# rccohn/AMPIS

Hardware: AMD Instinct MI355X
Metric: images/sec Mask R-CNN R50-FPN @1024x1024 inference (higher is better)
Workload: dtype f32 (convs: f16x3 split-operand MFMA -- 22-bit operands, exact products, fp32 accumulate); 1 GPU; BASELINE configs[1]: R50-FPN inference, batch=8 synthetic 1024x1024 micrographs per GPU, K=2, 1000 proposals/img, TEST.DETECTIONS_PER_IMAGE=200, seeded random-init weights, outputs on the host: boxes, scores, classes and every mask as its COCO compressed-RLE counts string (encoded on the device); batch_per_gpu=8, global_batch=8, parallelism=image-parallel replicas x1, no data-path collective

## Files before the change

ampis_amd/_lib.py:

```python
import ctypes as C
import os

_HERE = os.path.dirname(os.path.abspath(__file__))
LIB_PATH = os.path.join(_HERE, "lib", "libampis_hip.so")


class AmpError(RuntimeError):
    pass


class ConvDesc(C.Structure):
    _fields_ = [(n, C.c_int) for n in
                ("B", "H", "W", "Cin", "Cout", "KH", "KW", "stride", "pad", "relu", "res_mode", "out_mode")]


class RpnLevels(C.Structure):
    _fields_ = [("nlevels", C.c_int), ("A", C.c_int), ("ld", C.c_int), ("pred", C.c_void_p * 5),
                ("h", C.c_int * 5), ("w", C.c_int * 5), ("stride", C.c_int * 5), ("anchor_size", C.c_int * 5)]


class FpnFeats(C.Structure):
    _fields_ = [("feat", C.c_void_p * 4), ("h", C.c_int * 4), ("w", C.c_int * 4), ("stride", C.c_int * 4),
                ("C", C.c_int)]

# ... 66 lines not shown
        "amp_prof_launches": ([vp, C.POINTER(ProfLaunch), i, C.POINTER(i)], i),
        "amp_timer_stop": ([vp, C.POINTER(f)], i),
        "amp_destroy": ([vp], None),
        "amp_sync": ([vp], i),
        "amp_malloc": ([vp, C.c_size_t, C.POINTER(vp)], i),
        "amp_free": ([vp, vp], i),
        "amp_memcpy_h2d": ([vp, vp, vp, C.c_size_t], i),
        "amp_memcpy_d2h": ([vp, vp, vp, C.c_size_t], i),
        "amp_memset": ([vp, vp, i, C.c_size_t], i),
        "amp_conv2d_nhwc": ([vp, C.POINTER(ConvDesc), vp, vp, vp, vp, vp, vp], i),
        "amp_conv2d_nhwc_ex": ([vp, C.POINTER(ConvDesc), vp, vp, vp, vp, vp, vp, vp], i),
        "amp_conv2d_nhwc_fmt": ([vp, C.POINTER(ConvDesc), vp, vp, vp, vp, vp, vp, i], i),
        "amp_unsplit_rows": ([vp, vp, C.c_longlong, i, vp], i),
        "amp_group_expand_weights": ([vp, vp, i, i, i, i, vp], i),
        "amp_resize_scratch_bytes": ([i, i, i, i], C.c_size_t),
        "amp_resize_bilinear_u8": ([vp, vp, i, i, vp, i, i, vp], i),
        "amp_resize_flip_u8": ([vp, vp, i, i, vp, i, i, i, i, vp], i),
        "amp_compact_dets": ([vp, i, i, vp, vp, vp, vp, vp, vp, vp, vp], i),
        "amp_set_conv_mode": ([vp, i], i),
        "amp_get_conv_mode": ([vp], i),
        "amp_conv_range_flag": ([vp, i, C.POINTER(C.c_int)], i),
        "amp_split_weights": ([vp, vp, C.c_longlong, i, vp], i),
        "amp_bottleneck64_tail": ([vp, i, i, i, vp, vp, vp, vp, vp, vp, vp, i, vp, vp], i),
        "amp_conv2d_grouped_nhwc": ([vp, C.POINTER(ConvDesc), i, vp, vp, vp, vp, vp, vp], i),
        "amp_conv2d_grouped_nhwc_fmt": ([vp, C.POINTER(ConvDesc), i, vp, vp, vp, vp, vp, vp, i], i),
        "amp_conv_wgrad_scratch_floats": ([C.POINTER(ConvDesc)], C.c_size_t),
        "amp_conv2d_wgrad": ([vp, C.POINTER(ConvDesc), vp, vp, vp, vp, vp, i], i),
        "amp_conv2d_wgrad_scaled": ([vp, C.POINTER(ConvDesc), vp, vp, vp, vp, vp, i, i, i], i),
        "amp_colsum": ([vp, vp, i, i, vp, vp, i], i),
        "amp_dgrad_weights": ([vp, vp, vp, i, i, i, i, vp], i),
        "amp_dgrad_weights_split": ([vp, vp, vp, i, i, i, i, vp], i),
        "amp_preprocess": ([vp, vp, i, i, i, i, i, C.POINTER(f), C.POINTER(f), vp, vp], i),
        "amp_model_set_image_sizes": ([vp, vp, i], i),
        "amp_maxpool3x3s2": ([vp, vp, i, i, i, i, vp], i),
        "amp_subsample2": ([vp, vp, i, i, i, i, vp], i),
        "amp_rpn_topk": ([vp, C.POINTER(RpnLevels), i, i, vp, i, vp, vp, vp], i),
        "amp_rpn_decode": ([vp, C.POINTER(RpnLevels), i, i, vp, vp, vp, i, i, i, vp, vp, vp], i),
        "amp_rpn_decode_sized": ([vp, C.POINTER(RpnLevels), i, i, vp, vp, vp, i, i, vp, i, vp, vp, vp], i),
        "amp_sort_gather": ([vp, i, i, i, vp, vp, vp, vp, vp, vp, vp, vp, vp], i),
        "amp_sort_gather_n": ([vp, i, i, i, vp, vp, vp, vp, vp, vp, vp, vp, vp, vp], i),
        "amp_nms": ([vp, i, i, vp, vp, vp, f, i, vp, vp, vp], i),
        "amp_rpn_nms_scratch_words": ([i, i, i], C.c_size_t),
        "amp_rpn_nms_levels": ([vp, i, i, i, i, vp, vp, vp, f, i, vp, vp, vp, vp, vp, vp, vp], i),
        "amp_roi_align": ([vp, C.POINTER(FpnFeats), vp, vp, vp, i, i, vp, vp], i),
        "amp_roi_align_fmt": ([vp, C.POINTER(FpnFeats), vp, vp, vp, i, i, vp, vp, i], i),
        "amp_box_candidates": ([vp, vp, i, vp, vp, i, i, i, C.POINTER(f), f, i, i, vp, vp, i, vp, vp], i),
# ... 239 lines not shown
```

ampis_amd/csrc/common.h:

```cpp
#pragma once
#include <hip/hip_runtime.h>
#ifdef __HIPCC__
#include <hip/hip_ext.h>
#endif
#include <stdint.h>
#include <stdio.h>
#include <algorithm>
#include <string>

#include "../../include/ampis_hip.h"

namespace amp {

void set_error(const char* fmt, ...);

#define AMP_HIP_CHECK(expr)                                                         \
    do {                                                                            \
        hipError_t _e = (expr);                                                     \
        if (_e != hipSuccess) {                                                     \
            amp::set_error("%s:%d: %s -> %s", __FILE__, __LINE__, #expr,            \
                           hipGetErrorString(_e));                                  \
            return AMP_ERR_HIP;                                                     \
        }                                                                           \
    } while (0)
// ... 152 lines not shown
                       float* dense_boxes, unsigned long long* keys, int ccap, int* cand_count, int* overflow);
struct WeightJob {
    const float* w;
    const float* scale;
    unsigned int* out;
    int N, KH, KW, C;
    int transpose;
};
int weight_jobs_run(amp_ctx* ctx, const WeightJob* jobs_dev, const void* chunks_dev, int nchunks);
int sgd_chunks_run(amp_ctx* ctx, const unsigned long long* chunks_dev, int nchunks, float* p, const float* g, float* v, float lr,
                   float momentum, float weight_decay, float grad_scale);
int wgrad_async_begin(amp_ctx* ctx, float* scratch1);
int wgrad_async_join(amp_ctx* ctx);
int wgrad_async_end(amp_ctx* ctx);
int roi_align_bwd_run(amp_ctx* ctx, float* const dfeat[4], const int fh[4], const int fw[4], const int stride[4], int C, const float* rois,
                      const int* batch_idx, int R, int P, const float* dout, int B, int init);
int upsample2_bwd_run(amp_ctx* ctx, const float* dfine, float* dcoarse, int B, int Hc, int Wc, int C, int init);
int maxpool_run(amp_ctx* ctx, const float* x, int B, int H, int W, int C, float* y, int y_split);
int compact_dets_run(amp_ctx* ctx, int B, int D, const int* det_count, const float* det_boxes, const float* det_scores, const int* det_classes,
                     float* boxes, float* scores, int* classes, int* batch, int* n_total );
int stem_pool_run(amp_ctx* ctx, int B, int H, int W, const float* x, int x_split, const float* w_split, const float* scale, const float* shift,
                  float* pool, int pool_split);
int conv_c64_fused3_run(amp_ctx* ctx, int B, int H, int W, const float* x_split, const float* w2_split, const float* scale2, const float* shift2,
                        const float* w3_split, const float* scale3, const float* shift3, int C3, const float* res_split, float* y_split);
bool stem_pool_applies(amp_ctx* ctx, const float* w_split);
bool stem_u8_applies(amp_ctx* ctx, const float* w_split);
int stem_pool_u8_run(amp_ctx* ctx, const uint8_t* img, int B, int H, int W, int Hp, int Wp, const float mean[3], const float std_[3],
                     const int* img_hw, const float* w_split, const float* scale, const float* shift, float* pool, int pool_split);
int preprocess_run(amp_ctx* ctx, const uint8_t* img_bgr, int B, int H, int W, int Hp, int Wp, const float mean[3], const float std[3],
                   const int* img_hw, float* out, int out_split);
}
```

ampis_amd/csrc/conv.hip:

```cpp
#include "common.h"
#include <type_traits>

namespace {

typedef float f32x4 __attribute__((ext_vector_type(4)));
typedef float f32x16 __attribute__((ext_vector_type(16)));
typedef _Float16 f16x8 __attribute__((ext_vector_type(8)));
typedef _Float16 f16x2 __attribute__((ext_vector_type(2)));
typedef _Float16 f16x4 __attribute__((ext_vector_type(4)));
typedef unsigned int u32x4 __attribute__((ext_vector_type(4)));
constexpr float LO_SCALE = 2048.0f;

constexpr int BK = 32;
constexpr int LDS_LD = 36;

struct ConvArgs {
    const float* x;
    const float* w;
    const float* scale;
    const float* shift;
    const float* res;
    const float* mask;
    float* y;
    int B, H, W, Cin;
// ... 345 lines not shown
                }
                if (a.relu) o = fmaxf(o, 0.f);
                const _Float16 hh = (_Float16)o;
                hi[q] = hh;
                lo[q] = (_Float16)((o - (float)hh) * LO_SCALE);
            }
            if (mv[t]) {
                char* base = reinterpret_cast<char*>(a.y + yrow[t]) + col_b;
                *reinterpret_cast<f16x8*>(base) = hi;
                *reinterpret_cast<f16x8*>(base + 64) = lo;
            }
        }
        if (CHECK && bad) atomicOr(a.range_flag, 1);
    }
}

__device__ __forceinline__ int swap_channel(int w) {
    const int j = w >> 4, q = (w >> 2) & 3, e = w & 3;
    return 32 * (j >> 1) + 8 * q + 4 * (j & 1) + e;
}

typedef float f32x2 __attribute__((ext_vector_type(2)));

template <bool SPATIAL, bool CHECK, int MBR, bool AFFINE_LDS = false, bool PLAIN = false>
__device__ __forceinline__ void conv_epilogue_direct_rows(const ConvArgs& a, f32x4 (&acc)[MBR][4], int lane, const int (&mrow_in)[MBR], int nw0,
                                                          const float* lsc = nullptr, const float* lsh = nullptr, int nrel0 = 0) {
    const int lq = lane >> 4;
    const bool has_res = !PLAIN && a.res_mode != 0, has_mask = !PLAIN && a.mask != nullptr;
    const bool deconv = SPATIAL && a.out_mode == 1;
    const int C2 = a.Cout >> 2;
    const int tap = deconv ? nw0 / C2 : 0, ncol0 = deconv ? nw0 - tap * C2 : nw0;
    const int yld = deconv ? C2 : a.Cout;
    f32x2 sc[2][4], sh[2][4];
    size_t colb[2];
#pragma unroll
    for (int g = 0; g < 2; ++g) {
        const int n = nw0 + 32 * g + 8 * lq;
        const int nc = ncol0 + 32 * g + 8 * lq;
        colb[g] = (size_t)(nc >> 5) * 128 + (size_t)(nc & 31) * 2;
#pragma unroll
        for (int p = 0; p < 4; ++p) {
            if constexpr (AFFINE_LDS) {
                const int nr = nrel0 + 32 * g + 8 * lq + 2 * p;
                sc[g][p] = f32x2{lsc[nr], lsc[nr + 1]};
                sh[g][p] = f32x2{lsh[nr], lsh[nr + 1]};
            } else {
                sc[g][p] = a.scale ? f32x2{a.scale[n + 2 * p], a.scale[n + 2 * p + 1]} : f32x2{1.f, 1.f};
                sh[g][p] = a.shift ? f32x2{a.shift[n + 2 * p], a.shift[n + 2 * p + 1]} : f32x2{0.f, 0.f};
            }
// ... 78 lines not shown
                f32x2 o = v * sc[g][p] + sh[g][p];
                if (has_res) {
                    const f32x2 r1 = {(float)rh[g][2 * p], (float)rh[g][2 * p + 1]};
                    const f32x2 r2 = {(float)rl[g][2 * p], (float)rl[g][2 * p + 1]};
                    o = o + (r1 + r2 * (1.0f / LO_SCALE));
                }
                if (a.relu) { o[0] = fmaxf(o[0], 0.f); o[1] = fmaxf(o[1], 0.f); }
                if (has_mask) {
                    const f32x2 mk = f32x2{(float)mh[g][2 * p], (float)mh[g][2 * p + 1]} + f32x2{(float)ml[g][2 * p], (float)ml[g][2 * p + 1]} * (1.0f / LO_SCALE);
                    o[0] = mk[0] > 0.f ? o[0] : 0.f;
                    o[1] = mk[1] > 0.f ? o[1] : 0.f;
                }
                const f16x2 h = __builtin_convertvector(o, f16x2);
                const f32x2 hf = {(float)h[0], (float)h[1]};
                const f32x2 l = __builtin_elementwise_fma(hf, f32x2{-LO_SCALE, -LO_SCALE}, o * LO_SCALE);
                const f16x2 lh = __builtin_convertvector(l, f16x2);
                hi[2 * p] = h[0]; hi[2 * p + 1] = h[1];
                lo[2 * p] = lh[0]; lo[2 * p + 1] = lh[1];
            }
            if (mv) {
                char* base = reinterpret_cast<char*>(a.y + yrow) + colb[g];
                *reinterpret_cast<f16x8*>(base) = hi;
                *reinterpret_cast<f16x8*>(base + 64) = lo;
            }
        }
    }
    if (CHECK && (!(chk[0] == 0.f) || !(chk[1] == 0.f))) atomicOr(a.range_flag, 1);
}

template <bool SPATIAL, bool CHECK>
__device__ __forceinline__ void conv_epilogue_direct(const ConvArgs& a, f32x4 (&acc)[4][4], int lane, int mw0, int nw0) {
    const int l15 = lane & 15;
    const int mrows[4] = {mw0 + l15, mw0 + 16 + l15, mw0 + 32 + l15, mw0 + 48 + l15};
    conv_epilogue_direct_rows<SPATIAL, CHECK, 4>(a, acc, lane, mrows, nw0);
}

template <int WTM, int WTN, bool SPATIAL, bool CHECK>
__device__ __forceinline__ void conv_epilogue_swapped(const ConvArgs& a, f32x4 (&acc)[4][4], float* lds, int wave, int lane, int mw0, int nw0) {
    const int l15 = lane & 15, lq = lane >> 4;
    constexpr int SLD = WTN + 4;
    float* stage = lds + wave * (WTM * SLD);
#pragma unroll
    for (int i = 0; i < 4; ++i)
#pragma unroll
        for (int j = 0; j < 4; ++j)
            *reinterpret_cast<f32x4*>(stage + (i * 16 + l15) * SLD + 32 * (j >> 1) + 8 * lq + 4 * (j & 1)) = acc[i][j];
// ... 1395 lines not shown
            int mrows[2];
#pragma unroll
            for (int i = 0; i < 2; ++i) {
                const int oy = oyw + 2 * h + i, ox = ox0 + l15;
                mrows[i] = (oy < a.Ho && ox < a.Wo) ? (b * a.Ho + oy) * a.Wo + ox : a.M;
            }
            conv_epilogue_direct_rows<false, true, 2>(a, reinterpret_cast<f32x4 (&)[2][4]>(acc[2 * h]), lane, mrows, n0 + wn * 64);
        }
    }
#ifdef AMP_STAMP
    if (lane == 0)
        for (int q = 0; q < 8; ++q) atomicAdd(&g_stamp[wave * 8 + q], (unsigned long long)st_acc[q]);
#endif
}

struct Fuse3Args {
    const float* w3;
    const float* scale3;
    const float* shift3;
    const float* res;
    float* y;
    int C3;
    unsigned int w3_bytes;
};
template <bool DIAG, bool FUSE3 = false>
__global__ __launch_bounds__(256, 2) void conv3x3_c64_kernel(const ConvArgs a, const unsigned int x_bytes, const unsigned int w_bytes, const int tiles_x, const int tiles_y, const Fuse3Args f3) {
    constexpr int TH = 8, TW = 16, PH = TH + 2, PW = TW + 2, NPIX = PH * PW;
    constexpr int ROWF = 64;
    constexpr int NINST = NPIX / 4;
    static_assert(NPIX % 4 == 0, "patch pixels per DMA instruction");
    __shared__ __attribute__((aligned(16))) float lds[NPIX * ROWF + 2 * 64 * ROWF];
    float* patch = lds;
    float* wbuf = lds + NPIX * ROWF;
    const int tid = threadIdx.x, lane = tid & 63;
    const int wave = __builtin_amdgcn_readfirstlane(tid >> 6);
    const int l15 = lane & 15, lq = lane >> 4;
    int t = amp::xcd_remap(blockIdx.x, a.nblk);
    const int tile_n = t % a.ntn; t /= a.ntn;
    const int tx = t % tiles_x; t /= tiles_x;
    const int ty = t % tiles_y;
    const int b = t / tiles_y;
    const int oy0 = ty * TH, ox0 = tx * TW, n0 = tile_n * 64;
    const int cwin = a.grouped ? n0 : 0;
    const __amdgpu_buffer_rsrc_t rsrc_x = __builtin_amdgcn_make_buffer_rsrc(const_cast<float*>(a.x), 0, x_bytes, 0x00020000);
    const __amdgpu_buffer_rsrc_t rsrc_w = __builtin_amdgcn_make_buffer_rsrc(const_cast<float*>(a.w), 0, w_bytes, 0x00020000);
    const int sub = lane >> 4, chunk = lane & 15;
    for (int it = wave; it < NINST; it += 4) {
        const int q = it * 4 + sub;
        const int py = q / PW, px = q - py * PW;
        const int iy = oy0 - 1 + py, ix = ox0 - 1 + px;
        const bool v = (unsigned)iy < (unsigned)a.H && (unsigned)ix < (unsigned)a.W;
        const unsigned int voff = v ? (unsigned int)((((size_t)(b * a.H + iy) * a.W + ix) * a.Cin + cwin) * 4 + (size_t)((chunk ^ (q & 15)) * 16)) : OOB_VOFF;
        __builtin_amdgcn_raw_ptr_buffer_load_lds(rsrc_x, (__attribute__((address_space(3))) void*)(patch + it * 4 * ROWF), 16, (int)voff, 0, 0, 0);
    }
// ... 91 lines not shown
                    chk = __builtin_elementwise_fma(v, f32x2{0.f, 0.f}, chk);
                    f32x2 o = v * sc[p] + sh[p];
                    if (a.relu) { o[0] = fmaxf(o[0], 0.f); o[1] = fmaxf(o[1], 0.f); }
                    const f16x2 h = __builtin_convertvector(o, f16x2);
                    const f32x2 hf = {(float)h[0], (float)h[1]};
                    const f32x2 l = __builtin_elementwise_fma(hf, f32x2{-LO_SCALE, -LO_SCALE}, o * LO_SCALE);
                    const f16x2 lh = __builtin_convertvector(l, f16x2);
                    t2h[i][g][2 * p] = h[0]; t2h[i][g][2 * p + 1] = h[1];
                    t2l[i][g][2 * p] = lh[0]; t2l[i][g][2 * p + 1] = lh[1];
                }
            }
        }
        if (!(chk[0] == 0.f) || !(chk[1] == 0.f)) atomicOr(a.range_flag, 1);
        __syncthreads();
        const __amdgpu_buffer_rsrc_t rsrc_w3 = __builtin_amdgcn_make_buffer_rsrc(const_cast<float*>(f3.w3), 0, f3.w3_bytes, 0x00020000);
        float* w3s = lds;
        const int ninst3 = f3.C3 / 4;
        for (int it = wave; it < ninst3; it += 4) {
            const int r = it * 4 + sub;
            const int n = (r & ~63) + swap_channel(r & 63);
            const unsigned int voff = (unsigned int)((size_t)n * 256 + (size_t)((chunk ^ (r & 15)) * 16));
            __builtin_amdgcn_raw_ptr_buffer_load_lds(rsrc_w3, (__attribute__((address_space(3))) void*)(w3s + it * 4 * ROWF), 16, (int)voff, 0, 0, 0);
        }
        __syncthreads();
        ConvArgs a3 = a;
        a3.scale = f3.scale3; a3.shift = f3.shift3; a3.res = f3.res; a3.mask = nullptr; a3.y = f3.y;
        a3.Cout = f3.C3; a3.relu = 1; a3.res_mode = 1; a3.res_split = 1; a3.y_split = 1; a3.out_mode = 0; a3.mask_split = 0;
        for (int c = 0; c < f3.C3 / 64; ++c) {
            f32x4 acc3[2][4], acx3[2][4];
#pragma unroll
            for (int i = 0; i < 2; ++i)
#pragma unroll
                for (int j = 0; j < 4; ++j)
#pragma unroll
                    for (int e = 0; e < 4; ++e) { acc3[i][j][e] = 0.f; acx3[i][j][e] = 0.f; }
            const float* wc = w3s + c * 64 * ROWF;
#pragma unroll
            for (int g = 0; g < 2; ++g) {
                F16x3Frags<2, 4> f;
#pragma unroll
                for (int i = 0; i < 2; ++i) { f.ah[i] = t2h[i][g]; f.al[i] = t2l[i][g]; }
#pragma unroll
                for (int j = 0; j < 4; ++j) {
                    const float* row = wc + (j * 16 + l15) * ROWF;
                    f.bh[j] = *reinterpret_cast<const f16x8*>(row + 4 * ((8 * g + lq) ^ l15));
                    f.bl[j] = *reinterpret_cast<const f16x8*>(row + 4 * ((8 * g + 4 + lq) ^ l15));
                }
                f16x3_mfma16<2, 4, true>(f, acc3, acx3);
            }
#pragma unroll
            for (int i = 0; i < 2; ++i)
#pragma unroll
                for (int j = 0; j < 4; ++j)
#pragma unroll
                    for (int e = 0; e < 4; ++e) acc3[i][j][e] = __fadd_rn(acc3[i][j][e], __fmul_rn(acx3[i][j][e], 1.0f / LO_SCALE));
            conv_epilogue_direct_rows<false, true, 2>(a3, acc3, lane, mrows, 64 * c);
        }
    }
}


template <bool SCALED>
__device__ __forceinline__ void split8(const f32x4& v0, const f32x4& v1, f16x8& hi, f16x8& lo, float in_scale) {
#pragma unroll
    for (int j = 0; j < 8; ++j) {
        float x = j < 4 ? v0[j] : v1[j - 4];
        if (SCALED) x *= in_scale;
        const _Float16 h = (_Float16)x;
        hi[j] = h;
        lo[j] = (_Float16)((x - (float)h) * LO_SCALE);
    }
}

template <int BN, int EPI, bool STEM = false, bool SCALED = false>
__global__ __launch_bounds__(BN == 256 ? 512 : 256, BN == 256 ? 1 : 2) void conv_f16x3_kernel(const ConvArgs a, const unsigned int x_bytes,
                                                                                                const unsigned int w_bytes) {
    constexpr int BM = 128;
    constexpr int WTM = BM / 2, WTN = (BN == 64) ? 32 : 64;
    constexpr int NWN = BN / WTN, NW = 2 * NWN;
// ... 1215 lines not shown
            launch_glds<64, false>(a, epi, ctx->stream, (unsigned int)x_bytes, (unsigned int)w_bytes);
        }
    } else if (a.Cout > 64) {
        a.ntn = amp::cdiv(a.Cout, 128);
        a.nblk = ntm * a.ntn;
        switch (g_conv_ablate) {
            case 1: AMP_TIMED_LAUNCH((conv_mfma_kernel<BM, 128, 1>), dim3(a.nblk), dim3(256), 0, ctx->stream, a); break;
            case 2: AMP_TIMED_LAUNCH((conv_mfma_kernel<BM, 128, 2>), dim3(a.nblk), dim3(256), 0, ctx->stream, a); break;
            case 3: AMP_TIMED_LAUNCH((conv_mfma_kernel<BM, 128, 3>), dim3(a.nblk), dim3(256), 0, ctx->stream, a); break;
            default: AMP_TIMED_LAUNCH((conv_mfma_kernel<BM, 128, 0>), dim3(a.nblk), dim3(256), 0, ctx->stream, a);
        }
    } else {
        a.ntn = 1;
        a.nblk = ntm;
        AMP_TIMED_LAUNCH((conv_mfma_kernel<BM, 64>), dim3(a.nblk), dim3(256), 0, ctx->stream, a);
    }
    AMP_HIP_CHECK(hipGetLastError());
    return AMP_OK;
}


static int g_fuse23 = getenv("AMP_NO_FUSE23") ? 0 : 1;
extern "C" void amp_debug_set_fuse23(int v) { g_fuse23 = v; }
int amp::conv_c64_fused3_run(amp_ctx* ctx, int B, int H, int W, const float* x_split, const float* w2_split, const float* scale2, const float* shift2,
                             const float* w3_split, const float* scale3, const float* shift3, int C3, const float* res_split, float* y_split) {
    if (!g_fuse23 || g_patch_conv == 0 || !g_direct_epi || ctx->conv_mode != AMP_CONV_F16X3 || !w2_split || !w3_split) return 1;
    if (C3 % 64 != 0 || C3 > 256 || B < 1 || H < 1 || W < 1) return 1;
    const size_t x_bytes = (size_t)B * H * W * 64 * sizeof(float), w_bytes = (size_t)64 * 576 * sizeof(float), r_bytes = (size_t)B * H * W * C3 * sizeof(float);
    const long long tiles = (long long)B * amp::cdiv(H, 8) * amp::cdiv(W, 16);
    if (x_bytes >= (size_t)OOB_VOFF || r_bytes >= ((size_t)1 << 32) || (long long)B * H * W >= (1ll << 29) / 4 || (g_patch_conv != 2 && tiles < 512)) return 1;
    ConvArgs a = ConvArgs();
    a.x = x_split; a.w = w2_split; a.scale = scale2; a.shift = shift2;
    a.B = B; a.H = H; a.W = W; a.Cin = 64; a.Cout = 64; a.KH = 3; a.KW = 3; a.stride = 1; a.pad = 1; a.Ho = H; a.Wo = W;
    a.M = B * H * W; a.K = 576; a.nsteps = 18; a.cin_win = 64; a.grouped = 0;
    a.relu = 1; a.in_scale = a.out_scale = 1.0f; a.y_split = 1; a.direct_epi = 1;
    a.range_flag = ctx->d_conv_flag;
    a.ntn = 1; a.nblk = (int)tiles;
    set_fastdiv((unsigned int)(a.Ho * a.Wo), &a.div_howo_mul, &a.div_howo_shr);
    set_fastdiv((unsigned int)a.Wo, &a.div_wo_mul, &a.div_wo_shr);
    Fuse3Args f3;
    f3.w3 = w3_split; f3.scale3 = scale3; f3.shift3 = shift3; f3.res = res_split; f3.y = y_split; f3.C3 = C3; f3.w3_bytes = (unsigned int)((size_t)C3 * 64 * sizeof(float));
    amp_prof_rec* rec = nullptr;
    if (ctx->prof_on) {
        if (ctx->prof_used < ctx->prof_pool.size()) {
            rec = &ctx->prof_pool[ctx->prof_used++];
            rec->flops = 2.0 * (double)a.M * (64.0 * 576.0 + (double)C3 * 64.0);
            rec->variant = 1;
            rec->bytes = (double)x_bytes + (double)w_bytes + (double)f3.w3_bytes + 2.0 * (double)r_bytes;
            rec->M = a.M; rec->N = C3; rec->K = 576 + 64;
        } else {
            ctx->prof_truncated = true;
        }
    }
    amp::ProfLaunchScope timed(rec ? rec->e0 : nullptr, rec ? rec->e1 : nullptr);
    AMP_TIMED_LAUNCH((conv3x3_c64_kernel<false, true>), dim3(a.nblk), dim3(256), 0, ctx->stream, a, (unsigned int)x_bytes, (unsigned int)w_bytes, amp::cdiv(W, 16), amp::cdiv(H, 8), f3);
    AMP_HIP_CHECK(hipGetLastError());
    return AMP_OK;
}

extern "C" int amp_bottleneck64_tail(amp_ctx* ctx, int B, int H, int W, const float* x_split, const float* w2_split, const float* scale2, const float* shift2,
                                     const float* w3_split, const float* scale3, const float* shift3, int C3, const float* res_split, float* y_split) {
    AMP_REQUIRE(ctx && x_split && w2_split && w3_split && res_split && y_split, "%s", "amp_bottleneck64_tail: null argument");
    const int st = amp::conv_c64_fused3_run(ctx, B, H, W, x_split, w2_split, scale2, shift2, w3_split, scale3, shift3, C3, res_split, y_split);
    if (st == 1) { amp::set_error("amp_bottleneck64_tail: the fused kernel does not apply (AMP_CONV_F16X3, C3 %% 64 == 0, C3 <= 256, >= 512 tiles of 8 x 16)"); return AMP_ERR_STATE; }
    return st;
}
```

ampis_amd/csrc/model.hip:

```cpp
#include <math.h>
#include <string.h>

#include <map>
#include <string>
#include <vector>

#include "common.h"

namespace {

struct ConvW {
    float* w = nullptr;
    float* scale = nullptr;
    float* shift = nullptr;
    int cout = 0, cin = 0, kh = 0, kw = 0;
    float* w_split = nullptr;
    float* wt_split = nullptr;
    float w_absmax = 0.f;
    int groups = 1;
};

struct NamedBuf {
    void* ptr;
    int dtype;
// ... 287 lines not shown
    AMP_ALLOC(stem, float, (size_t)B * h * w * 64);
    const int h4 = (h + 2 - 3) / 2 + 1, w4 = (w + 2 - 3) / 2 + 1;
    AMP_ALLOC(pool, float, (size_t)B * h4 * w4 * 64);
    if (!dry) {
        const ConvW& sw = CONV("backbone.bottom_up.stem.conv1");
        int fused = 1;
        if (stem_from_u8)
            fused = amp::stem_pool_u8_run(ctx, imgs_d, B, H, W, Hp, Wp, c.pixel_mean, c.pixel_std, T.img_hw, sw.w_split, sw.scale, sw.shift, pool, native_all ? 1 : 0);
        else if (sw.cin == 4 && sw.kw == 8 && sw.kh == 7 && sw.cout == 64 && !m->split_stale)
            fused = amp::stem_pool_run(ctx, B, Hp, Wp, x0, x0_split ? 1 : 0, sw.w_split, sw.scale, sw.shift, pool, native_all ? 1 : 0);
        if (fused < 0) return fused;
        if (fused == 1 && x0_split) { amp::set_error("amp_model: the input was split for the fused stem, which then did not launch"); return AMP_ERR_STATE; }
        if (fused == 1) {
            AMP_TRY(launch_conv(m, sw, x0, B, Hp, Wp, 2, 3, true, 0, nullptr, 0, stem));
            AMP_TRY(amp::maxpool_run(ctx, stem, B, h, w, 64, pool, native_all ? 1 : 0));
        }
    }
    if (!dry) tap(m, "stem_pool", pool, native_all ? SPL : 0, {B, h4, w4, 64});

    float* cur = pool;
    int ch = h4, cw_ = w4;
    float* res_out[4];
    int res_h[4], res_w[4];
    for (int s = 0; s < 4; ++s) {
        for (int b = 0; b < m->nblk[s]; ++b) {
            const std::string p = std::string("backbone.bottom_up.") + kStage[s] + "." + std::to_string(b);
            const int st = (b == 0) ? kStride[s] : 1;
            const int oh = (ch - 1) / st + 1, ow = (cw_ - 1) / st + 1;
            const size_t mark = ws.off;
            AMP_ALLOC(out, float, (size_t)B * oh * ow * kOut[s]);
            const size_t keep = ws.off;
            const float* shortcut = cur;
            if (b == 0) {
                AMP_ALLOC(sc, float, (size_t)B * oh * ow * kOut[s]);
                if (!dry) AMP_TRY(launch_conv(m, CONV((p + ".shortcut").c_str()), cur, B, ch, cw_, st, 0, false, 0, nullptr, 0, sc, FMT(native_all, native_all, false)));
                shortcut = sc;
            }
            const int st1 = c.stride_in_1x1 ? st : 1, st2 = c.stride_in_1x1 ? 1 : st;
            const int h1 = (ch - 1) / st1 + 1, w1 = (cw_ - 1) / st1 + 1;
            AMP_ALLOC(t1, float, (size_t)B * h1 * w1 * m->mid[s]);
            AMP_ALLOC(t2, float, (size_t)B * oh * ow * m->mid[s]);
            if (!dry) {
                const bool t1s = reads_split(p + ".conv2"), t2s = reads_split(p + ".conv3");
                AMP_TRY(launch_conv(m, CONV((p + ".conv1").c_str()), cur, B, ch, cw_, st1, 0, true, 0, nullptr, 0, t1, FMT(native_all, t1s, false)));
                int fused23 = 1;
                const ConvW &c2w = CONV((p + ".conv2").c_str()), &c3w = CONV((p + ".conv3").c_str());
                if (s == 0 && t1s && t2s && native_all && st2 == 1 && c2w.groups == 1 && c2w.cin == 64 && c2w.cout == 64 && c2w.kh == 3 && c3w.cin == 64 && c3w.kh == 1 &&
                    !m->split_stale && c2w.scale && c3w.scale)
                    fused23 = amp::conv_c64_fused3_run(ctx, B, oh, ow, t1, c2w.w_split, c2w.scale, c2w.shift, c3w.w_split, c3w.scale, c3w.shift, c3w.cout, shortcut, out);
                if (fused23 < 0) return fused23;
                if (fused23 == 1) {
                    AMP_TRY(launch_conv(m, c2w, t1, B, h1, w1, st2, 1, true, 0, nullptr, 0, t2, FMT(t1s, t2s, false)));
                    AMP_TRY(launch_conv(m, c3w, t2, B, oh, ow, 1, 0, true, 1, shortcut, 0, out, FMT(t2s, native_all, native_all)));
                }
            }
            (void)mark;
            if (m->saving) {
                amp_model::BlockAct ba;
                ba.key = p; ba.x_in = cur; ba.t1 = t1; ba.t2 = t2; ba.sc = (b == 0) ? const_cast<float*>(shortcut) : nullptr; ba.out = out;
                ba.in_h = ch; ba.in_w = cw_; ba.oh = oh; ba.ow = ow; ba.cin = (b == 0) ? (s == 0 ? 64 : kOut[s - 1]) : kOut[s];
                ba.mid = m->mid[s]; ba.cout = kOut[s]; ba.stride = st; ba.stage = s; ba.has_sc = (b == 0);
                if (!dry) m->blocks.push_back(ba);
            } else {
                ws.off = keep;
            }
            cur = out;
            ch = oh; cw_ = ow;
        }
        res_out[s] = cur; res_h[s] = ch; res_w[s] = cw_;
        if (!dry) tap(m, kStage[s], cur, native_all ? SPL : 0, {B, ch, cw_, kOut[s]});
    }

    float* feat[5];
    int fh[5], fw[5];
    const int fstride[5] = {4, 8, 16, 32, 64};
    float* prev_lat = nullptr;
    for (int l = 5; l >= 2; --l) {
        const int s = l - 2;
        const std::string ln = "backbone.fpn_lateral" + std::to_string(l), on = "backbone.fpn_output" + std::to_string(l);
        AMP_ALLOC(lat, float, (size_t)B * res_h[s] * res_w[s] * 256);
        AMP_ALLOC(outp, float, (size_t)B * res_h[s] * res_w[s] * 256);
        if (!dry) {
            AMP_TRY(launch_conv(m, CONV(ln.c_str()), res_out[s], B, res_h[s], res_w[s], 1, 0, false, prev_lat ? 2 : 0, prev_lat, 0, lat,
                                FMT(native_all, native_all, native_all && prev_lat != nullptr)));
            AMP_TRY(launch_conv(m, CONV(on.c_str()), lat, B, res_h[s], res_w[s], 1, 1, false, 0, nullptr, 0, outp, FMT(native_all, native_all, false)));
        }
        prev_lat = lat;
        m->lat[s] = lat;
// ... 1914 lines not shown
```

ampis_amd/ops.py:

```python
import ctypes as C

import torch

from . import _lib
from ._lib import ConvDesc, check, lib, ptr


def torch_context(device=0):
    if not torch.cuda.is_available():
        raise _lib.AmpError("no HIP device visible: the ampis_amd hot path has no CPU fallback")
    with torch.cuda.device(device):
        return _lib.Context(device, borrow_stream=torch.cuda.current_stream().cuda_stream)


def _f32c(t):
    assert t is None or (t.is_cuda and t.dtype == torch.float32 and t.is_contiguous()), "need contiguous fp32 CUDA tensor"
    return t


FMT_X_SPLIT, FMT_Y_SPLIT, FMT_RES_SPLIT = 1, 2, 4


def split_rows(ctx, t):
    _f32c(t)
# ... 29 lines not shown
    else:
        y = torch.empty((B, Ho, Wo, Cout), device=x.device, dtype=torch.float32)
    if fmt:
        assert mask is None
        check(lib().amp_conv2d_nhwc_fmt(ctx.handle, C.byref(d), ptr(x), ptr(w), ptr(scale), ptr(shift), ptr(res), ptr(y), int(fmt)),
              "amp_conv2d_nhwc_fmt")
        return y
    check(lib().amp_conv2d_nhwc_ex(ctx.handle, C.byref(d), ptr(x), ptr(w), ptr(scale), ptr(shift), ptr(res), ptr(_f32c(mask)), ptr(y)),
          "amp_conv2d_nhwc_ex")
    return y


def bottleneck64_tail(ctx, x_split, w2, scale2, shift2, w3, scale3, shift3, res_split):
    _f32c(x_split), _f32c(w2), _f32c(w3), _f32c(res_split)
    B, H, W, _ = x_split.shape
    C3 = w3.shape[0]
    w2s, w3s = split_rows(ctx, w2.reshape(64, 576)), split_rows(ctx, w3.reshape(C3, 64))
    y = torch.empty((B, H, W, C3), device=x_split.device, dtype=torch.float32)
    check(lib().amp_bottleneck64_tail(ctx.handle, B, H, W, ptr(x_split), ptr(w2s), ptr(_f32c(scale2)), ptr(_f32c(shift2)), ptr(w3s), ptr(_f32c(scale3)),
                                      ptr(_f32c(shift3)), C3, ptr(res_split), ptr(y)), "amp_bottleneck64_tail")
    return y


def conv2d_grouped_nhwc(ctx, x, w, groups, scale=None, shift=None, res=None, stride=1, pad=0, relu=False, fmt=0):
    _f32c(x), _f32c(w), _f32c(scale), _f32c(shift), _f32c(res)
    B, H, W, Cin = x.shape
    Cout, KH, KW, cpg = w.shape
    assert Cin == Cout and cpg * groups == Cin
    w_win = torch.empty((Cout, KH, KW, 64), device=x.device, dtype=torch.float32)
    check(lib().amp_group_expand_weights(ctx.handle, ptr(w), Cout, KH, KW, cpg, ptr(w_win)), "amp_group_expand_weights")
    Ho = (H + 2 * pad - KH) // stride + 1
    Wo = (W + 2 * pad - KW) // stride + 1
    d = ConvDesc(B, H, W, Cin, Cout, KH, KW, stride, pad, int(relu), 0 if res is None else 1, 0)
    y = torch.empty((B, Ho, Wo, Cout), device=x.device, dtype=torch.float32)
    if fmt:
        check(lib().amp_conv2d_grouped_nhwc_fmt(ctx.handle, C.byref(d), int(groups), ptr(x), ptr(w_win), ptr(scale), ptr(shift), ptr(res), ptr(y), int(fmt)),
              "amp_conv2d_grouped_nhwc_fmt")
        return y
    check(lib().amp_conv2d_grouped_nhwc(ctx.handle, C.byref(d), int(groups), ptr(x), ptr(w_win), ptr(scale), ptr(shift), ptr(res), ptr(y)),
          "amp_conv2d_grouped_nhwc")
    return y


def resize_bilinear_u8(ctx, img, h, w):
    import numpy as np
    img = np.ascontiguousarray(img, dtype=np.uint8)
# ... 210 lines not shown
```

include/ampis_hip.h:

```cpp
#ifndef AMPIS_HIP_H
#define AMPIS_HIP_H

#include <stddef.h>
#include <stdint.h>

#ifdef __cplusplus
extern "C" {
#endif

typedef enum amp_status {
    AMP_OK = 0,
    AMP_ERR_ARG = -1,
    AMP_ERR_HIP = -2,
    AMP_ERR_NOMEM = -3,
    AMP_ERR_STATE = -4
} amp_status;

typedef struct amp_ctx amp_ctx;

const char* amp_last_error(void);
int  amp_version(void);
#define AMP_STREAM_BORROW 1
int  amp_init(int device, void* hip_stream, int flags, amp_ctx** out);
void amp_destroy(amp_ctx* ctx);
// ... 45 lines not shown
} amp_conv_desc;
int amp_conv2d_nhwc(amp_ctx* ctx, const amp_conv_desc* d, const float* x, const float* w,
                    const float* scale, const float* shift, const float* res, float* y);
int amp_group_expand_weights(amp_ctx* ctx, const float* w, int Cout, int KH, int KW, int cpg, float* w_win);
int amp_conv2d_grouped_nhwc(amp_ctx* ctx, const amp_conv_desc* d, int groups, const float* x, const float* w_win,
                            const float* scale, const float* shift, const float* res, float* y);
int amp_conv2d_grouped_nhwc_fmt(amp_ctx* ctx, const amp_conv_desc* d, int groups, const float* x, const float* w_win,
                                const float* scale, const float* shift, const float* res, float* y, int fmt);
size_t amp_grouped_wgrad_scratch_floats(const amp_conv_desc* d);
int amp_conv2d_grouped_wgrad(amp_ctx* ctx, const amp_conv_desc* d, int groups, const float* x, const float* dy, const float* scale,
                             float* scratch, float* grad_win);
int amp_conv2d_grouped_wgrad_fmt(amp_ctx* ctx, const amp_conv_desc* d, int groups, const float* x, const float* dy, const float* scale,
                                 float* scratch, float* grad_win, int fmt, int dy_shift);
int amp_group_dgrad_weights(amp_ctx* ctx, const float* w_win, const float* scale, int C, int KH, int KW, float* wt_win);
int amp_conv2d_nhwc_ex(amp_ctx* ctx, const amp_conv_desc* d, const float* x, const float* w, const float* scale, const float* shift,
                       const float* res, const float* mask, float* y);

enum { AMP_FMT_X_SPLIT = 1, AMP_FMT_Y_SPLIT = 2, AMP_FMT_RES_SPLIT = 4, AMP_FMT_MASK_SPLIT = 8 };
int amp_conv2d_nhwc_fmt(amp_ctx* ctx, const amp_conv_desc* d, const float* x, const float* w, const float* scale, const float* shift,
                        const float* res, float* y, int fmt);
int amp_unsplit_rows(amp_ctx* ctx, const float* x_split, long long rows, int C, float* out);
int amp_bottleneck64_tail(amp_ctx* ctx, int B, int H, int W, const float* x_split, const float* w2_split, const float* scale2, const float* shift2,
                          const float* w3_split, const float* scale3, const float* shift3, int C3, const float* res_split, float* y_split);

size_t amp_conv_wgrad_scratch_floats(const amp_conv_desc* d);
int amp_conv2d_wgrad(amp_ctx* ctx, const amp_conv_desc* d, const float* x, const float* dy, const float* scale, float* scratch,
                     float* grad, int accumulate);
int amp_conv2d_wgrad_scaled(amp_ctx* ctx, const amp_conv_desc* d, const float* x, const float* dy, const float* scale, float* scratch,
                            float* grad, int accumulate, int dy_shift, int x_shift);
int amp_conv2d_wgrad_fmt(amp_ctx* ctx, const amp_conv_desc* d, const float* x, const float* dy, const float* scale, float* scratch,
                            float* grad, int accumulate, int dy_shift, int x_shift, int x_split, float* bias_grad, int bias_accumulate);
int amp_colsum(amp_ctx* ctx, const float* dy, int M, int N, float* scratch, float* out, int accumulate);
int amp_colsum_split(amp_ctx* ctx, const float* dy, int M, int N, float* scratch, float* out, int accumulate, float* dy_split, int shift);
int amp_colsum_of_split(amp_ctx* ctx, const float* dy_split, int M, int N, float* scratch, float* out, int accumulate, int shift);
int amp_dgrad_weights(amp_ctx* ctx, const float* w, const float* scale, int Cout, int KH, int KW, int Cin, float* wt);
int amp_dgrad_weights_split(amp_ctx* ctx, const float* w, const float* scale, int Cout, int KH, int KW, int Cin, float* wt_split);
int amp_roi_align_bwd(amp_ctx* ctx, float* const dfeat[4], const int fh[4], const int fw[4], const int stride[4], int C, const float* rois,
                      const int* batch_idx, int R, int P, const float* dout);
int amp_roi_align_bwd_batched(amp_ctx* ctx, float* const dfeat[4], const int fh[4], const int fw[4], const int stride[4], int C, const float* rois,
                              const int* batch_idx, int R, int P, const float* dout, int B);
int amp_upsample2_bwd(amp_ctx* ctx, const float* dfine, float* dcoarse, int B, int Hc, int Wc, int C);
int amp_subsample2_bwd(amp_ctx* ctx, const float* dy, float* dx, int B, int H, int W, int C);
int amp_relu_mask(amp_ctx* ctx, float* g, const float* act, size_t n);
int amp_relu_mask_split(amp_ctx* ctx, float* g, const float* act_split, size_t n, int C);
int amp_relu_mask_to_split(amp_ctx* ctx, const float* g, const float* act_split, float* out_split, size_t n, int C, int shift);
int amp_subsample2_bwd_split(amp_ctx* ctx, const float* dy_split, float* dx, int B, int H, int W, int C, int shift);
// ... 246 lines not shown
```

Measured before the change: 497.0 images/s.

## Chain next block's conv1 into fused conv2+conv3 bottleneck tail kernel

The fused stage-0 bottleneck tail kernel (conv2 3x3 + conv3 1x1 + residual) can now also compute the next block's 1x1 conv1. It does this by keeping each 64-channel output slice in registers and accumulating it against conv1 weights streamed into LDS behind the conv3 weights. The model loop hands the next block a precomputed t1 buffer and skips its conv1 launch. This saves one launch and one full re-read of the block output per chained block, at the cost of more registers, extra LDS, and an added barrier per channel chunk, which could reduce occupancy.

```diff
diff --git a/ampis_amd/_lib.py b/ampis_amd/_lib.py
--- a/ampis_amd/_lib.py
+++ b/ampis_amd/_lib.py
@@ -112,6 +112,8 @@
         "amp_conv_range_flag": ([vp, i, C.POINTER(C.c_int)], i),
         "amp_split_weights": ([vp, vp, C.c_longlong, i, vp], i),
         "amp_bottleneck64_tail": ([vp, i, i, i, vp, vp, vp, vp, vp, vp, vp, i, vp, vp], i),
+        "amp_bottleneck64_tail_chain": ([vp, i, i, i, vp, vp, vp, vp, vp, vp, vp, i, vp, vp, vp, vp, vp, vp], i),
+        "amp_debug_set_conv1_chain": ([i], None),
         "amp_conv2d_grouped_nhwc": ([vp, C.POINTER(ConvDesc), i, vp, vp, vp, vp, vp, vp], i),
         "amp_conv2d_grouped_nhwc_fmt": ([vp, C.POINTER(ConvDesc), i, vp, vp, vp, vp, vp, vp, i], i),
         "amp_conv_wgrad_scratch_floats": ([C.POINTER(ConvDesc)], C.c_size_t),
diff --git a/ampis_amd/csrc/common.h b/ampis_amd/csrc/common.h
--- a/ampis_amd/csrc/common.h
+++ b/ampis_amd/csrc/common.h
@@ -198,7 +198,8 @@
 int stem_pool_run(amp_ctx* ctx, int B, int H, int W, const float* x, int x_split, const float* w_split, const float* scale, const float* shift,
                   float* pool, int pool_split);
 int conv_c64_fused3_run(amp_ctx* ctx, int B, int H, int W, const float* x_split, const float* w2_split, const float* scale2, const float* shift2,
-                        const float* w3_split, const float* scale3, const float* shift3, int C3, const float* res_split, float* y_split);
+                        const float* w3_split, const float* scale3, const float* shift3, int C3, const float* res_split, float* y_split,
+                        const float* w1_split = nullptr, const float* scale1 = nullptr, const float* shift1 = nullptr, float* t1_split = nullptr);
 bool stem_pool_applies(amp_ctx* ctx, const float* w_split);
 bool stem_u8_applies(amp_ctx* ctx, const float* w_split);
 int stem_pool_u8_run(amp_ctx* ctx, const uint8_t* img, int B, int H, int W, int Hp, int Wp, const float mean[3], const float std_[3],
diff --git a/ampis_amd/csrc/conv.hip b/ampis_amd/csrc/conv.hip
--- a/ampis_amd/csrc/conv.hip
+++ b/ampis_amd/csrc/conv.hip
@@ -391,9 +391,10 @@
 
 typedef float f32x2 __attribute__((ext_vector_type(2)));
 
-template <bool SPATIAL, bool CHECK, int MBR, bool AFFINE_LDS = false, bool PLAIN = false>
+template <bool SPATIAL, bool CHECK, int MBR, bool AFFINE_LDS = false, bool PLAIN = false, bool KEEP = false>
 __device__ __forceinline__ void conv_epilogue_direct_rows(const ConvArgs& a, f32x4 (&acc)[MBR][4], int lane, const int (&mrow_in)[MBR], int nw0,
-                                                          const float* lsc = nullptr, const float* lsh = nullptr, int nrel0 = 0) {
+                                                          const float* lsc = nullptr, const float* lsh = nullptr, int nrel0 = 0,
+                                                          f16x8 (*kh)[2] = nullptr, f16x8 (*kl)[2] = nullptr) {
     const int lq = lane >> 4;
     const bool has_res = !PLAIN && a.res_mode != 0, has_mask = !PLAIN && a.mask != nullptr;
     const bool deconv = SPATIAL && a.out_mode == 1;
@@ -518,6 +519,10 @@
                 char* base = reinterpret_cast<char*>(a.y + yrow) + colb[g];
                 *reinterpret_cast<f16x8*>(base) = hi;
                 *reinterpret_cast<f16x8*>(base + 64) = lo;
+            }
+            if constexpr (KEEP) {
+                kh[i][g] = mv ? hi : f16x8{};
+                kl[i][g] = mv ? lo : f16x8{};
             }
         }
     }
@@ -1959,14 +1964,22 @@
     float* y;
     int C3;
     unsigned int w3_bytes;
+    const float* w1;
+    const float* scale1;
+    const float* shift1;
+    float* t1;
+    unsigned int w1_bytes;
 };
-template <bool DIAG, bool FUSE3 = false>
+template <bool DIAG, bool FUSE3 = false, bool CHAIN = false>
 __global__ __launch_bounds__(256, 2) void conv3x3_c64_kernel(const ConvArgs a, const unsigned int x_bytes, const unsigned int w_bytes, const int tiles_x, const int tiles_y, const Fuse3Args f3) {
     constexpr int TH = 8, TW = 16, PH = TH + 2, PW = TW + 2, NPIX = PH * PW;
     constexpr int ROWF = 64;
     constexpr int NINST = NPIX / 4;
     static_assert(NPIX % 4 == 0, "patch pixels per DMA instruction");
-    __shared__ __attribute__((aligned(16))) float lds[NPIX * ROWF + 2 * 64 * ROWF];
+    static_assert(!CHAIN || FUSE3, "conv1 chains behind conv3");
+    constexpr int LDS_ROWS = CHAIN ? 256 + 64 : NPIX + 2 * 64;
+    static_assert(NPIX + 2 * 64 <= LDS_ROWS && LDS_ROWS * ROWF * 4 <= 80 * 1024, "LDS budget: two workgroups per CU");
+    __shared__ __attribute__((aligned(16))) float lds[LDS_ROWS * ROWF];
     float* patch = lds;
     float* wbuf = lds + NPIX * ROWF;
     const int tid = threadIdx.x, lane = tid & 63;
@@ -2104,11 +2117,31 @@
             const unsigned int voff = (unsigned int)((size_t)n * 256 + (size_t)((chunk ^ (r & 15)) * 16));
             __builtin_amdgcn_raw_ptr_buffer_load_lds(rsrc_w3, (__attribute__((address_space(3))) void*)(w3s + it * 4 * ROWF), 16, (int)voff, 0, 0, 0);
         }
+        const __amdgpu_buffer_rsrc_t rsrc_w1 = __builtin_amdgcn_make_buffer_rsrc(const_cast<float*>(f3.w1), 0, f3.w1_bytes, 0x00020000);
+        auto stage_w1 = [&](int c, float* dst) {
+#pragma unroll
+            for (int g = 0; g < 4; ++g) {
+                const int r = (wave * 4 + g) * 4 + sub;
+                const unsigned int voff = (unsigned int)(((size_t)swap_channel(r) * f3.C3 + (size_t)c * 64) * 4 + (size_t)((chunk ^ (r & 15)) * 16));
+                __builtin_amdgcn_raw_ptr_buffer_load_lds(rsrc_w1, (__attribute__((address_space(3))) void*)(dst + (wave * 4 + g) * 4 * ROWF), 16, (int)voff, 0, 0, 0);
+            }
+        };
+        if constexpr (CHAIN) stage_w1(0, lds + 256 * ROWF);
         __syncthreads();
         ConvArgs a3 = a;
         a3.scale = f3.scale3; a3.shift = f3.shift3; a3.res = f3.res; a3.mask = nullptr; a3.y = f3.y;
         a3.Cout = f3.C3; a3.relu = 1; a3.res_mode = 1; a3.res_split = 1; a3.y_split = 1; a3.out_mode = 0; a3.mask_split = 0;
-        for (int c = 0; c < f3.C3 / 64; ++c) {
+        f32x4 acc1[2][4], acx1[2][4];
+        if constexpr (CHAIN) {
+#pragma unroll
+            for (int i = 0; i < 2; ++i)
+#pragma unroll
+                for (int j = 0; j < 4; ++j)
+#pragma unroll
+                    for (int e = 0; e < 4; ++e) { acc1[i][j][e] = 0.f; acx1[i][j][e] = 0.f; }
+        }
+        const int nch = f3.C3 / 64;
+        for (int c = 0; c < nch; ++c) {
             f32x4 acc3[2][4], acx3[2][4];
 #pragma unroll
             for (int i = 0; i < 2; ++i)
@@ -2130,13 +2163,48 @@
                 }
                 f16x3_mfma16<2, 4, true>(f, acc3, acx3);
             }
+            if constexpr (CHAIN) {
+                __syncthreads();
+                if (c + 1 < nch) stage_w1(c + 1, w3s + c * 64 * ROWF);
+            }
 #pragma unroll
             for (int i = 0; i < 2; ++i)
 #pragma unroll
                 for (int j = 0; j < 4; ++j)
 #pragma unroll
                     for (int e = 0; e < 4; ++e) acc3[i][j][e] = __fadd_rn(acc3[i][j][e], __fmul_rn(acx3[i][j][e], 1.0f / LO_SCALE));
-            conv_epilogue_direct_rows<false, true, 2>(a3, acc3, lane, mrows, 64 * c);
+            if constexpr (!CHAIN) {
+                conv_epilogue_direct_rows<false, true, 2>(a3, acc3, lane, mrows, 64 * c);
+            } else {
+                f16x8 yh[2][2], yl[2][2];
+                conv_epilogue_direct_rows<false, true, 2, false, false, true>(a3, acc3, lane, mrows, 64 * c, nullptr, nullptr, 0, yh, yl);
+                const float* w1c = c == 0 ? lds + 256 * ROWF : w3s + (c - 1) * 64 * ROWF;
+#pragma unroll
+                for (int g = 0; g < 2; ++g) {
+                    F16x3Frags<2, 4> f;
+#pragma unroll
+                    for (int i = 0; i < 2; ++i) { f.ah[i] = yh[i][g]; f.al[i] = yl[i][g]; }
+#pragma unroll
+                    for (int j = 0; j < 4; ++j) {
+                        const float* row = w1c + (j * 16 + l15) * ROWF;
+                        f.bh[j] = *reinterpret_cast<const f16x8*>(row + 4 * ((8 * g + lq) ^ l15));
+                        f.bl[j] = *reinterpret_cast<const f16x8*>(row + 4 * ((8 * g + 4 + lq) ^ l15));
+                    }
+                    f16x3_mfma16<2, 4, true>(f, acc1, acx1);
+                }
+            }
+        }
+        if constexpr (CHAIN) {
+#pragma unroll
+            for (int i = 0; i < 2; ++i)
+#pragma unroll
+                for (int j = 0; j < 4; ++j)
+#pragma unroll
+                    for (int e = 0; e < 4; ++e) acc1[i][j][e] = __fadd_rn(acc1[i][j][e], __fmul_rn(acx1[i][j][e], 1.0f / LO_SCALE));
+            ConvArgs a1 = a;
+            a1.scale = f3.scale1; a1.shift = f3.shift1; a1.res = nullptr; a1.mask = nullptr; a1.y = f3.t1;
+            a1.Cout = 64; a1.relu = 1; a1.res_mode = 0; a1.res_split = 0; a1.y_split = 1; a1.out_mode = 0; a1.mask_split = 0;
+            conv_epilogue_direct_rows<false, true, 2>(a1, acc1, lane, mrows, 0);
         }
     }
 }
@@ -3398,10 +3466,15 @@
 
 static int g_fuse23 = getenv("AMP_NO_FUSE23") ? 0 : 1;
 extern "C" void amp_debug_set_fuse23(int v) { g_fuse23 = v; }
+static int g_conv1_chain = getenv("AMP_NO_CONV1_CHAIN") ? 0 : 1;
+extern "C" void amp_debug_set_conv1_chain(int v) { g_conv1_chain = v; }
 int amp::conv_c64_fused3_run(amp_ctx* ctx, int B, int H, int W, const float* x_split, const float* w2_split, const float* scale2, const float* shift2,
-                             const float* w3_split, const float* scale3, const float* shift3, int C3, const float* res_split, float* y_split) {
+                             const float* w3_split, const float* scale3, const float* shift3, int C3, const float* res_split, float* y_split,
+                             const float* w1_split, const float* scale1, const float* shift1, float* t1_split) {
     if (!g_fuse23 || g_patch_conv == 0 || !g_direct_epi || ctx->conv_mode != AMP_CONV_F16X3 || !w2_split || !w3_split) return 1;
     if (C3 % 64 != 0 || C3 > 256 || B < 1 || H < 1 || W < 1) return 1;
+    const bool chain = w1_split != nullptr;
+    if (chain && (!g_conv1_chain || !t1_split)) return 1;
     const size_t x_bytes = (size_t)B * H * W * 64 * sizeof(float), w_bytes = (size_t)64 * 576 * sizeof(float), r_bytes = (size_t)B * H * W * C3 * sizeof(float);
     const long long tiles = (long long)B * amp::cdiv(H, 8) * amp::cdiv(W, 16);
     if (x_bytes >= (size_t)OOB_VOFF || r_bytes >= ((size_t)1 << 32) || (long long)B * H * W >= (1ll << 29) / 4 || (g_patch_conv != 2 && tiles < 512)) return 1;
@@ -3416,20 +3489,24 @@
     set_fastdiv((unsigned int)a.Wo, &a.div_wo_mul, &a.div_wo_shr);
     Fuse3Args f3;
     f3.w3 = w3_split; f3.scale3 = scale3; f3.shift3 = shift3; f3.res = res_split; f3.y = y_split; f3.C3 = C3; f3.w3_bytes = (unsigned int)((size_t)C3 * 64 * sizeof(float));
+    f3.w1 = w1_split; f3.scale1 = scale1; f3.shift1 = shift1; f3.t1 = t1_split; f3.w1_bytes = chain ? f3.w3_bytes : 0;
     amp_prof_rec* rec = nullptr;
     if (ctx->prof_on) {
         if (ctx->prof_used < ctx->prof_pool.size()) {
             rec = &ctx->prof_pool[ctx->prof_used++];
-            rec->flops = 2.0 * (double)a.M * (64.0 * 576.0 + (double)C3 * 64.0);
+            rec->flops = 2.0 * (double)a.M * (64.0 * 576.0 + (double)C3 * 64.0 * (chain ? 2.0 : 1.0));
             rec->variant = 1;
-            rec->bytes = (double)x_bytes + (double)w_bytes + (double)f3.w3_bytes + 2.0 * (double)r_bytes;
-            rec->M = a.M; rec->N = C3; rec->K = 576 + 64;
+            rec->bytes = (double)x_bytes + (double)w_bytes + (double)f3.w3_bytes + 2.0 * (double)r_bytes + (chain ? (double)f3.w1_bytes + (double)x_bytes : 0.0);
+            rec->M = a.M; rec->N = C3; rec->K = 576 + 64 + (chain ? C3 : 0);
         } else {
             ctx->prof_truncated = true;
         }
     }
     amp::ProfLaunchScope timed(rec ? rec->e0 : nullptr, rec ? rec->e1 : nullptr);
-    AMP_TIMED_LAUNCH((conv3x3_c64_kernel<false, true>), dim3(a.nblk), dim3(256), 0, ctx->stream, a, (unsigned int)x_bytes, (unsigned int)w_bytes, amp::cdiv(W, 16), amp::cdiv(H, 8), f3);
+    if (chain)
+        AMP_TIMED_LAUNCH((conv3x3_c64_kernel<false, true, true>), dim3(a.nblk), dim3(256), 0, ctx->stream, a, (unsigned int)x_bytes, (unsigned int)w_bytes, amp::cdiv(W, 16), amp::cdiv(H, 8), f3);
+    else
+        AMP_TIMED_LAUNCH((conv3x3_c64_kernel<false, true>), dim3(a.nblk), dim3(256), 0, ctx->stream, a, (unsigned int)x_bytes, (unsigned int)w_bytes, amp::cdiv(W, 16), amp::cdiv(H, 8), f3);
     AMP_HIP_CHECK(hipGetLastError());
     return AMP_OK;
 }
@@ -3441,3 +3518,13 @@
     if (st == 1) { amp::set_error("amp_bottleneck64_tail: the fused kernel does not apply (AMP_CONV_F16X3, C3 %% 64 == 0, C3 <= 256, >= 512 tiles of 8 x 16)"); return AMP_ERR_STATE; }
     return st;
 }
+
+extern "C" int amp_bottleneck64_tail_chain(amp_ctx* ctx, int B, int H, int W, const float* x_split, const float* w2_split, const float* scale2, const float* shift2,
+                                           const float* w3_split, const float* scale3, const float* shift3, int C3, const float* res_split, float* y_split,
+                                           const float* w1_split, const float* scale1, const float* shift1, float* t1_split) {
+    AMP_REQUIRE(ctx && x_split && w2_split && w3_split && res_split && y_split && w1_split && t1_split, "%s", "amp_bottleneck64_tail_chain: null argument");
+    const int st = amp::conv_c64_fused3_run(ctx, B, H, W, x_split, w2_split, scale2, shift2, w3_split, scale3, shift3, C3, res_split, y_split,
+                                            w1_split, scale1, shift1, t1_split);
+    if (st == 1) { amp::set_error("amp_bottleneck64_tail_chain: the chained kernel does not apply (the fused tail's conditions, the conv1 chain switched on)"); return AMP_ERR_STATE; }
+    return st;
+}
diff --git a/ampis_amd/csrc/model.hip b/ampis_amd/csrc/model.hip
--- a/ampis_amd/csrc/model.hip
+++ b/ampis_amd/csrc/model.hip
@@ -333,6 +333,8 @@
     int ch = h4, cw_ = w4;
     float* res_out[4];
     int res_h[4], res_w[4];
+    float* t1_pre = nullptr;
+    bool t1_done = false;
     for (int s = 0; s < 4; ++s) {
         for (int b = 0; b < m->nblk[s]; ++b) {
             const std::string p = std::string("backbone.bottom_up.") + kStage[s] + "." + std::to_string(b);
@@ -340,6 +342,11 @@
             const int oh = (ch - 1) / st + 1, ow = (cw_ - 1) / st + 1;
             const size_t mark = ws.off;
             AMP_ALLOC(out, float, (size_t)B * oh * ow * kOut[s]);
+            float* t1_next = nullptr;
+            if (s == 0 && b + 1 < m->nblk[s] && !m->saving) {
+                AMP_ALLOC(t1n, float, (size_t)B * oh * ow * m->mid[s]);
+                t1_next = t1n;
+            }
             const size_t keep = ws.off;
             const float* shortcut = cur;
             if (b == 0) {
@@ -349,16 +356,33 @@
             }
             const int st1 = c.stride_in_1x1 ? st : 1, st2 = c.stride_in_1x1 ? 1 : st;
             const int h1 = (ch - 1) / st1 + 1, w1 = (cw_ - 1) / st1 + 1;
-            AMP_ALLOC(t1, float, (size_t)B * h1 * w1 * m->mid[s]);
+            float* t1 = t1_pre;
+            if (!t1) {
+                AMP_ALLOC(t1a, float, (size_t)B * h1 * w1 * m->mid[s]);
+                t1 = t1a;
+            }
             AMP_ALLOC(t2, float, (size_t)B * oh * ow * m->mid[s]);
+            bool chained = false;
             if (!dry) {
                 const bool t1s = reads_split(p + ".conv2"), t2s = reads_split(p + ".conv3");
-                AMP_TRY(launch_conv(m, CONV((p + ".conv1").c_str()), cur, B, ch, cw_, st1, 0, true, 0, nullptr, 0, t1, FMT(native_all, t1s, false)));
+                if (!t1_done) AMP_TRY(launch_conv(m, CONV((p + ".conv1").c_str()), cur, B, ch, cw_, st1, 0, true, 0, nullptr, 0, t1, FMT(native_all, t1s, false)));
                 int fused23 = 1;
                 const ConvW &c2w = CONV((p + ".conv2").c_str()), &c3w = CONV((p + ".conv3").c_str());
                 if (s == 0 && t1s && t2s && native_all && st2 == 1 && c2w.groups == 1 && c2w.cin == 64 && c2w.cout == 64 && c2w.kh == 3 && c3w.cin == 64 && c3w.kh == 1 &&
-                    !m->split_stale && c2w.scale && c3w.scale)
-                    fused23 = amp::conv_c64_fused3_run(ctx, B, oh, ow, t1, c2w.w_split, c2w.scale, c2w.shift, c3w.w_split, c3w.scale, c3w.shift, c3w.cout, shortcut, out);
+                    !m->split_stale && c2w.scale && c3w.scale) {
+                    if (t1_next) {
+                        const std::string pn = std::string("backbone.bottom_up.") + kStage[s] + "." + std::to_string(b + 1);
+                        const ConvW& c1n = CONV((pn + ".conv1").c_str());
+                        if (reads_split(pn + ".conv1") && reads_split(pn + ".conv2") && c1n.groups == 1 && c1n.kh == 1 && c1n.kw == 1 && c1n.cin == c3w.cout &&
+                            c1n.cout == 64 && c1n.scale) {
+                            fused23 = amp::conv_c64_fused3_run(ctx, B, oh, ow, t1, c2w.w_split, c2w.scale, c2w.shift, c3w.w_split, c3w.scale, c3w.shift, c3w.cout, shortcut, out,
+                                                               c1n.w_split, c1n.scale, c1n.shift, t1_next);
+                            chained = fused23 == 0;
+                        }
+                    }
+                    if (!chained && fused23 >= 0)
+                        fused23 = amp::conv_c64_fused3_run(ctx, B, oh, ow, t1, c2w.w_split, c2w.scale, c2w.shift, c3w.w_split, c3w.scale, c3w.shift, c3w.cout, shortcut, out);
+                }
                 if (fused23 < 0) return fused23;
                 if (fused23 == 1) {
                     AMP_TRY(launch_conv(m, c2w, t1, B, h1, w1, st2, 1, true, 0, nullptr, 0, t2, FMT(t1s, t2s, false)));
@@ -375,6 +399,8 @@
             } else {
                 ws.off = keep;
             }
+            t1_pre = t1_next;
+            t1_done = chained;
             cur = out;
             ch = oh; cw_ = ow;
         }
diff --git a/ampis_amd/ops.py b/ampis_amd/ops.py
--- a/ampis_amd/ops.py
+++ b/ampis_amd/ops.py
@@ -75,6 +75,20 @@
     return y
 
 
+def bottleneck64_tail_chain(ctx, x_split, w2, scale2, shift2, w3, scale3, shift3, res_split, w1, scale1, shift1):
+    _f32c(x_split), _f32c(w2), _f32c(w3), _f32c(res_split), _f32c(w1)
+    B, H, W, _ = x_split.shape
+    C3 = w3.shape[0]
+    assert tuple(w1.shape) == (64, 1, 1, C3)
+    w2s, w3s, w1s = split_rows(ctx, w2.reshape(64, 576)), split_rows(ctx, w3.reshape(C3, 64)), split_rows(ctx, w1.reshape(64, C3))
+    y = torch.empty((B, H, W, C3), device=x_split.device, dtype=torch.float32)
+    t1 = torch.empty((B, H, W, 64), device=x_split.device, dtype=torch.float32)
+    check(lib().amp_bottleneck64_tail_chain(ctx.handle, B, H, W, ptr(x_split), ptr(w2s), ptr(_f32c(scale2)), ptr(_f32c(shift2)), ptr(w3s), ptr(_f32c(scale3)),
+                                            ptr(_f32c(shift3)), C3, ptr(res_split), ptr(y), ptr(w1s), ptr(_f32c(scale1)), ptr(_f32c(shift1)), ptr(t1)),
+          "amp_bottleneck64_tail_chain")
+    return y, t1
+
+
 def conv2d_grouped_nhwc(ctx, x, w, groups, scale=None, shift=None, res=None, stride=1, pad=0, relu=False, fmt=0):
     _f32c(x), _f32c(w), _f32c(scale), _f32c(shift), _f32c(res)
     B, H, W, Cin = x.shape
diff --git a/include/ampis_hip.h b/include/ampis_hip.h
--- a/include/ampis_hip.h
+++ b/include/ampis_hip.h
@@ -91,6 +91,10 @@
 int amp_unsplit_rows(amp_ctx* ctx, const float* x_split, long long rows, int C, float* out);
 int amp_bottleneck64_tail(amp_ctx* ctx, int B, int H, int W, const float* x_split, const float* w2_split, const float* scale2, const float* shift2,
                           const float* w3_split, const float* scale3, const float* shift3, int C3, const float* res_split, float* y_split);
+int amp_bottleneck64_tail_chain(amp_ctx* ctx, int B, int H, int W, const float* x_split, const float* w2_split, const float* scale2, const float* shift2,
+                                const float* w3_split, const float* scale3, const float* shift3, int C3, const float* res_split, float* y_split,
+                                const float* w1_split, const float* scale1, const float* shift1, float* t1_split);
+void amp_debug_set_conv1_chain(int on);
 
 size_t amp_conv_wgrad_scratch_floats(const amp_conv_desc* d);
 int amp_conv2d_wgrad(amp_ctx* ctx, const amp_conv_desc* d, const float* x, const float* dy, const float* scale, float* scratch,
```

New measurement: 500.0 images/s (median of 6 runs). No clear change (+0.6%).
